# matthieugomez/LeastSquaresOptim.jl

Hardware: AMD Instinct MI355X
Metric: lm_lsmr_outer_iterations_per_sec (higher is better)
Workload: dtype f64

## Files before the change

leastsquaresoptim.jl_amd/csrc/lsq_optimize.hip:

```cpp
#include <chrono>
#include <cmath>
#include <cstring>

#include "lsq_solver.h"
#include "lsq_spmv.h"

static constexpr double MIN_DELTA = 1e-16, MAX_DELTA = 1e16, MIN_STEP_QUALITY = 1e-3;
static constexpr double MIN_DIAGONAL = 1e-6, MAX_DIAGONAL = 1e32;
static constexpr double DECREASE_THRESHOLD = 0.25, INCREASE_THRESHOLD = 0.75;

enum { SL_GRAD = 8, SL_DX = 9, SL_NONFIN = 10, SL_TRIAL = 11, SL_PRED = 12, SL_SSR = 13, SL_W0 = 14, SL_W1 = 15,
       SL_W2 = 16, SL_SUM = 17 };

extern "C" int lsq_solver_create(lsq_ctx *c, lsq_mat *J, int kind, int for_lm, lsq_solver **out) {
    LSQ_RANGE("lsq_solver_create");
    if (!c || !J || !out) return LSQ_EARG;
    if (kind == LSQ_QR && J->kind != LSQ_MAT_DENSE) {
        lsq_set_error("solver QR() is not available for sparse Jacobians. Choose between Cholesky() and LSMR()");
        return LSQ_EARG;
    }
    const bool blockdiag = kind == LSQ_CHOLESKY && J->kind == LSQ_MAT_CSC && J->bd_blocks > 0;
    const bool bordered = kind == LSQ_CHOLESKY && J->kind == LSQ_MAT_CSC && J->br_blocks > 0;
    if (kind == LSQ_CHOLESKY && J->kind != LSQ_MAT_DENSE && !blockdiag && !bordered) {
        lsq_set_error("MethodError: no AbstractAllocatedSolver for Cholesky() with a sparse Jacobian "
// ... 351 lines not shown
    });
}

__global__ void __launch_bounds__(LSQ_NT)
k_wdot_slot(int n, const double *__restrict__ x, const double *__restrict__ y, const double *__restrict__ w,
            double *partials, unsigned *counter, double *out) {
    __shared__ double sh[LSQ_NT / 64];
    double acc = 0.0;
    for (int i = blockIdx.x * LSQ_NT + threadIdx.x; i < n; i += gridDim.x * LSQ_NT) acc += w[i] * x[i] * y[i];
    double b = block_sum<LSQ_NT>(acc, sh);
    grid_reduce<LSQ_NT>(b, partials, counter, gridDim.x, sh, [=](double t) { *out = t; });
}

__global__ void __launch_bounds__(LSQ_NT)
k_lincomb(int n, double a, const double *__restrict__ p, double b, const double *__restrict__ q,
          double *__restrict__ out) {
    for (int i = blockIdx.x * LSQ_NT + threadIdx.x; i < n; i += gridDim.x * LSQ_NT) {
        double v = p[i] * a;
        if (q) v += b * q[i];
        out[i] = v;
    }
}

static inline int ngrid(const lsq_ctx *c, long long n) {
    long long g = (n + LSQ_NT - 1) / LSQ_NT;
    long long cap = (long long)c->num_cus * 8;
    if (g > cap) g = cap;
    return g < 1 ? 1 : (int)g;
}

static int sumsq_to_slot(lsq_ctx *c, bool exact, long long n, const double *x, int ctr, double *d_out,
                         LsqSlotPublish pub = LsqSlotPublish()) {
    if (exact) return lsq_seq_reduce(c, 1, (int)n, x, nullptr, nullptr, d_out);
    long long g = (n + LSQ_NT - 1) / LSQ_NT, cap = (long long)c->num_cus * 2;
    if (g > cap) g = cap;
    if (g < 1) g = 1;
    LSQ_LAUNCH(k_sumsq_slot, dim3((int)g), dim3(LSQ_NT), 0, c->stream, n, x, c->d_partials, lsq_ctr(c, ctr), d_out,
                       pub);
    return LSQ_OK;
}
static int model_f(double *out, const double *x, void *user);
static int model_g(lsq_mat *J, const double *x, void *user);
static int model_f_sumsq(void *user, double *out, const double *x, int ctr, double *d_out, LsqSlotPublish pub, bool *done,
                         const int *skip = nullptr);
struct SpecGrad {
    int *gate;
    double ssr;
    double *grad;
    bool launched;
};
static int model_pair_tail(void *user, lsq_mat *J, const double *dx, const double *fcur, double *ftrial, const double *xt,
                           double *slot_pred, double *slot_trial, LsqSlotPublish pub, const int *skip, bool *done,
                           SpecGrad *sg = nullptr);
static void model_trial_buffers(void *user, const double *xt, double **t_out, double **s_out);
static int f_then_sumsq(lsq_ctx *c, bool exact, lsq_f_callback f, void *user, long long m, double *out, const double *x, int ctr,
                        double *d_out, LsqSlotPublish pub = LsqSlotPublish(), const int *skip = nullptr) {
    if (!exact && f == model_f) {
        bool fused = false;
        if (model_f_sumsq(user, out, x, ctr, d_out, pub, &fused, skip) != 0) {
            lsq_set_error("user callback reported failure");
            return LSQ_ECALLBACK;
        }
        if (fused) return LSQ_OK;
    } else if (f(out, x, user) != 0) {
        lsq_set_error("user callback reported failure");
        return LSQ_ECALLBACK;
    }
    return sumsq_to_slot(c, exact, m, out, ctr, d_out, pub);
}
static int predicted_to_slot(lsq_ctx *c, bool exact, lsq_mat *J, const double *d, const double *f, double *scratch,
                             int ctr, double *d_out, LsqSlotPublish pub = LsqSlotPublish(), const int *skip = nullptr);
static int wdot_to_slot(lsq_ctx *c, bool exact, int n, const double *x, const double *y, const double *w, int ctr,
                        double *d_out);
static int gradient_into(lsq_ctx *c, bool exact, lsq_mat *J, const double *f, double *g);

struct LoopBuffers {
    lsq_ctx *c;
    int m, n;
    double *dx = nullptr, *dtd = nullptr, *xt = nullptr, *ftrial = nullptr;
    double *dgn = nullptr, *dgr = nullptr, *grad = nullptr, *fpred = nullptr;
    double *lo = nullptr, *hi = nullptr;
    int *gate_ring = nullptr;
    int gate_next = 0;
    static constexpr int GATE_RING = 1024;
    ~LoopBuffers() {
        hipFree(gate_ring);
        hipFree(dx); hipFree(dtd); hipFree(xt); hipFree(ftrial); hipFree(dgn); hipFree(dgr); hipFree(grad); hipFree(fpred); hipFree(lo);
        hipFree(hi);
    }
};

struct LsqWorkspace {
    lsq_mat *J = nullptr;
    int m = 0, n = 0, optimizer = -1, solver_kind = -1;
    bool has_lo = false, has_hi = false;
    LoopBuffers *buf = nullptr;
    lsq_solver *solver = nullptr;
};
void lsq_workspace_free(void *p) {
    LsqWorkspace *w = (LsqWorkspace *)p;
    if (!w) return;
    delete w->buf;
    if (w->solver) lsq_solver_destroy(w->solver);
    delete w;
}

// ... 120 lines not shown
        return LSQ_ECALLBACK;
    }
    *ssr = v[0];
    *gnorm = v[1];
    *all_converged = v[2] > 0.5 ? 1 : 0;
    return LSQ_OK;
}

struct ShardedExit {
    lsq_ctx *c;
    const lsq_options *o;
    ShardedExit(lsq_ctx *c_, const lsq_options *o_) : c(c_), o(o_) {
        t_xchg_issued = 0;
        t_xchg_hook_failed = false;
    }
    int finish(int st) {
        c->idle_hook = nullptr;
        c->idle_user = nullptr;
        if (st != LSQ_OK && st != LSQ_ERCCL && o->allreduce && !t_xchg_hook_failed && t_xchg_issued < o->iterations) {
            double v[3] = {0.0, 0.0, -1.0};
            (void)o->allreduce(v, 3, o->allreduce_user);
        }
        return st;
    }
};

#define CB(call)                                          \
    do {                                                  \
        if ((call) != 0) {                                \
            lsq_set_error("user callback reported failure"); \
            return LSQ_ECALLBACK;                         \
        }                                                 \
    } while (0)

static int call_g(lsq_g_callback g, lsq_mat *J, const double *x, void *user) {
    J->version++;
    if (J->kind == LSQ_MAT_CSC && !J->d_cs_user) J->csr_fresh = false;
    CB(g(J, x, user));
    return lsq_ensure_csr(J);
}
int lsq_call_g(lsq_g_callback g, lsq_mat *J, const double *x, void *user) { return call_g(g, J, x, user); }

struct IterateGuard {
    lsq_ctx *c;
    double *&x, *&fcur;
    double *x_user, *fcur_user;
    int m, n;
    ~IterateGuard() {
        if (x != x_user) lsq_d2d(c, x_user, x, (size_t)n * sizeof(double));
        if (fcur != fcur_user) lsq_d2d(c, fcur_user, fcur, (size_t)m * sizeof(double));
    }
};

static int start_residual(lsq_ctx *c, lsq_mat *J, lsq_f_callback f, void *user, double *fcur, const double *x, double *ssr,
                          int *nonfinite_at) {
    const int m = J->m, n = J->n;
    if (lsq_small_mat(J) || lsq_small_vec(m) || m <= 0) {
        CB(f(fcur, x, user));
        LSQ_TRY(lsq_sumsq(c, m, fcur, ssr));
        return lsq_first_nonfinite(c, n, x, nonfinite_at);
    }
    static_assert(SL_TRIAL == SL_NONFIN + 1, "the two scalars of the loop head travel together");
    LSQ_TRY(lsq_first_nonfinite_to_slot(c, n, x, c->d_slots + SL_NONFIN));
    LSQ_TRY(f_then_sumsq(c, false, f, user, m, fcur, x, 7, c->d_slots + SL_TRIAL));
    double sl[2];
    LSQ_TRY(lsq_read_slots(c, SL_NONFIN, 2, sl));
    *nonfinite_at = (int)sl[0];
    *ssr = sl[1];
    return LSQ_OK;
}

static int optimize_lm_loop(lsq_ctx *c, lsq_solver *sv, LoopBuffers &b, lsq_mat *J, double *x_user, double *fcur_user,
                            lsq_f_callback f, lsq_g_callback g, void *user, const lsq_options *o, lsq_result *r);
static int optimize_lm(lsq_ctx *c, lsq_solver *sv, LoopBuffers &b, lsq_mat *J, double *x_user, double *fcur_user,
                       lsq_f_callback f, lsq_g_callback g, void *user, const lsq_options *o, lsq_result *r) {
    ShardedExit ex{c, o};
    return ex.finish(optimize_lm_loop(c, sv, b, J, x_user, fcur_user, f, g, user, o, r));
}
static int optimize_lm_loop(lsq_ctx *c, lsq_solver *sv, LoopBuffers &b, lsq_mat *J, double *x_user, double *fcur_user,
                            lsq_f_callback f, lsq_g_callback g, void *user, const lsq_options *o, lsq_result *r) {
    const int m = J->m, n = J->n;
    double *x = x_user, *fcur = fcur_user, *xt = b.xt, *ftrial = b.ftrial;
    IterateGuard guard{c, x, fcur, x_user, fcur_user, m, n};
    double delta = o->delta > 0 ? o->delta : 10.0;
    double decrease_factor = 2.0;
    int f_calls = 0, g_calls = 0, mul_calls = 0, xc = 0, fc = 0, gc = 0;
    bool converged = false;
    double ssr;
    int iter = 0, nonfinite_at = -1;
    const bool sharded = o->row_allreduce != nullptr;
    if (sharded) CB(f(fcur, x, user));
    else LSQ_TRY(start_residual(c, J, f, user, fcur, x, &ssr, &nonfinite_at));
    f_calls++;
    auto rows_sum = [&](double *d_buf, int count) -> int {
        if (o->row_allreduce(d_buf, count, (void *)c->stream, o->row_allreduce_user) != 0) {
            lsq_set_error("row all-reduce callback reported failure");
            return LSQ_ECALLBACK;
        }
        return LSQ_OK;
    };
    if (sharded) {
        LSQ_TRY(sumsq_to_slot(c, false, m, fcur, 7, c->d_slots + SL_TRIAL));
        LSQ_TRY(rows_sum(c->d_slots + SL_TRIAL, 1));
        LSQ_TRY(lsq_read_slots(c, SL_TRIAL, 1, &ssr));
        LSQ_TRY(lsq_first_nonfinite(c, n, x, &nonfinite_at));
    }
    r->ssr0 = ssr;
    double maxabs_gr = INFINITY;
    bool need_jac = true;
    const int gn = ngrid(c, n);
    const bool exact = lsq_small_mat(J) && !sharded && !(sv->kind == LSQ_LSMR && sv->gen_ldiv);
    int last_inner = 0;
    const bool no_spec_grad = getenv("LSQ_NO_SPEC_GRADIENT") != nullptr;
    bool spec_launched = false, spec_grad_ready = false, spec_pending = false;
    struct SpecGuard { lsq_mat *J; bool &ready; bool &pending; ~SpecGuard() { if (ready || pending) lsq_sparse_colsum_forget(J); } }
        spec_guard{J, spec_grad_ready, spec_pending};
    int local_done = 0;
    double gssr = ssr, ggr = maxabs_gr;
    long long inner_total = 0;
    while (iter < o->iterations) {
        if (!o->allreduce && converged) break;
        if (o->allreduce && converged) {
            int all = 1;
            gssr = ssr; ggr = maxabs_gr;
            LSQ_TRY(global_exchange(o, &gssr, &ggr, &all));
            if (all) break;
            ++iter; local_done = 1;
            continue;
        }
        iter++;
        if (nonfinite_at >= 0) {
            r->bad_index = nonfinite_at;
            r->iterations = iter - 1;
            lsq_set_error("IsFiniteException: non-finite x at index %d", nonfinite_at);
            return LSQ_ENONFINITE;
        }
        if (need_jac) {
            LSQ_TRY(call_g(g, J, x, user));
            g_calls++;
            need_jac = false;
        }
        bool have_grad = false;
        if (spec_grad_ready) {
            lsq_sparse_grad_colsum_adopt(J);
            have_grad = true;
// ... 129 lines not shown
        const double rho = pred_red > 0 ? (ssr - trial_ssr) / pred_red : 0.0;
        const bool accepted = rho > MIN_STEP_QUALITY;
        const bool dev_accepted = spec_launched && sl[5] != 0.0;
        spec_grad_ready = spec_launched && accepted && dev_accepted;
        if (spec_launched && dev_accepted && !accepted) lsq_sparse_colsum_forget(J);
        spec_pending = false;
        converged = assess(maxabs_dx, maxabs_gr, ssr, trial_ssr, o->x_tol, o->f_tol, o->g_tol, accepted, &xc, &fc, &gc);
        if (accepted) {
            std::swap(fcur, ftrial);
            std::swap(x, xt);
            ssr = trial_ssr;
            double q = 1.0 - (2.0 * rho - 1.0) * (2.0 * rho - 1.0) * (2.0 * rho - 1.0);
            delta = std::min(delta / std::max(1.0 / 3.0, q), MAX_DELTA);
            decrease_factor = 2.0;
            need_jac = true;
            nonfinite_at = trial_nonfinite;
        } else {
            LSQ_LAUNCH(k_revert, dim3(gn), dim3(LSQ_NT), 0, c->stream, n, xt, b.dx, x);
            nonfinite_at = trial_nonfinite;
            delta = std::max(delta / decrease_factor, MIN_DELTA);
            decrease_factor *= 2.0;
        }
        record(o, c, iter, n, ssr, maxabs_gr, delta, rho, lmiter, accepted ? 1 : 0, x);
    }
    (void)local_done;
    LSQ_HIP(hipStreamSynchronize(c->stream));
    r->optimizer = LSQ_LEVENBERG_MARQUARDT;
    r->ssr = o->allreduce ? gssr : ssr;
    r->iterations = iter;
    r->converged = converged; r->x_converged = xc; r->f_converged = fc; r->g_converged = gc;
    r->f_calls = f_calls; r->g_calls = g_calls; r->mul_calls = mul_calls;
    r->lsmr_iterations = inner_total;
    return LSQ_OK;
}

static int optimize_dogleg_loop(lsq_ctx *c, lsq_solver *sv, LoopBuffers &b, lsq_mat *J, double *x, double *fcur,
                                lsq_f_callback f, lsq_g_callback g, void *user, const lsq_options *o, lsq_result *r);
static int optimize_dogleg(lsq_ctx *c, lsq_solver *sv, LoopBuffers &b, lsq_mat *J, double *x, double *fcur,
                           lsq_f_callback f, lsq_g_callback g, void *user, const lsq_options *o, lsq_result *r) {
    ShardedExit ex{c, o};
    return ex.finish(optimize_dogleg_loop(c, sv, b, J, x, fcur, f, g, user, o, r));
}
static int optimize_dogleg_loop(lsq_ctx *c, lsq_solver *sv, LoopBuffers &b, lsq_mat *J, double *x_user, double *fcur_user,
                                lsq_f_callback f, lsq_g_callback g, void *user, const lsq_options *o, lsq_result *r) {
    const int m = J->m, n = J->n;
    double *x = x_user, *fcur = fcur_user, *xt = b.xt, *ftrial = b.ftrial;
    IterateGuard guard{c, x, fcur, x_user, fcur_user, m, n};
    double delta = o->delta > 0 ? o->delta : 1.0;
    bool reuse = false, converged = false;
    double wnorm_dgn = 0.0, wnorm_dgr = 0.0, alpha = 0.0, wdot_gr_gn = 0.0;
    int f_calls = 0, g_calls = 0, mul_calls = 0, xc = 0, fc = 0, gc = 0;
    double ssr;
    int iter = 0, nonfinite_at = -1;
    LSQ_TRY(start_residual(c, J, f, user, fcur, x, &ssr, &nonfinite_at));
    f_calls++;
    r->ssr0 = ssr;
    double maxabs_gr = INFINITY;
    const int gn = ngrid(c, n);
    const bool exact = lsq_small_mat(J);
    double gssr = ssr, ggr = maxabs_gr;
    long long inner_total = 0;
    while (iter < o->iterations) {
        if (!o->allreduce && converged) break;
        if (o->allreduce && converged) {
            int all = 1;
            gssr = ssr; ggr = maxabs_gr;
            LSQ_TRY(global_exchange(o, &gssr, &ggr, &all));
            if (all) break;
            ++iter;
            continue;
        }
        iter++;
        if (nonfinite_at >= 0) {
            r->bad_index = nonfinite_at;
            r->iterations = iter - 1;
            lsq_set_error("IsFiniteException: non-finite x at index %d", nonfinite_at);
            return LSQ_ENONFINITE;
        }
        int ls_iter = 0;
        bool exchanged = false;
        if (!reuse) {
            LSQ_TRY(call_g(g, J, x, user));
            g_calls++;
            bool have_grad = false;
            if (!exact && J->colsum_version != J->version && lsq_can_fuse_grad_colsum(J)) {
                LSQ_TRY(lsq_sparse_grad_colsum(J, fcur, b.dgr));
                have_grad = true;
            }
            const double *cs = lsq_cached_colsum(J);
            if (!cs) return LSQ_EHIP;
            LSQ_LAUNCH(k_dl_scale, dim3(gn), dim3(LSQ_NT), 0, c->stream, n, cs, b.dtd);
            if (iter == 1) {
                double wx2;
                LSQ_TRY(lsq_wdot(c, n, x, x, b.dtd, &wx2));
                double wx = std::sqrt(wx2);
                if (wx > 0) delta *= wx;
            }
            if (!have_grad) LSQ_TRY(gradient_into(c, exact, J, fcur, b.dgr));
            mul_calls++;
            LSQ_LAUNCH(k_gradnorm, dim3(gn), dim3(LSQ_NT), 0, c->stream, n, b.dgr, x, b.lo, b.hi,
                               c->d_partials, lsq_ctr(c, 4), c->d_slots + SL_GRAD);
            LSQ_TRY(lsq_ediv(c, n, b.dgr, b.dtd, b.dgr));
            LSQ_TRY(wdot_to_slot(c, exact, n, b.dgr, b.dgr, b.dtd, 5, c->d_slots + SL_W0));
            LSQ_TRY(predicted_to_slot(c, exact, J, b.dgr, nullptr, b.fpred, 6, c->d_slots + SL_SUM));
            mul_calls++;
            LSQ_TRY(lsq_fill(c, n, 0.0, b.dgn));
            if (o->allreduce) {
// ... 85 lines not shown
    r->iterations = iter;
    r->converged = converged; r->x_converged = xc; r->f_converged = fc; r->g_converged = gc;
    r->f_calls = f_calls; r->g_calls = g_calls; r->mul_calls = mul_calls;
    r->lsmr_iterations = inner_total;
    return LSQ_OK;
}

extern "C" int lsq_optimize(lsq_ctx *c, int optimizer, int solver_kind, lsq_mat *J, double *x, double *fcur,
                            lsq_f_callback f, lsq_g_callback g, void *user, const lsq_options *opt, lsq_result *res) {
    LSQ_RANGE("lsq_optimize");
    if (!c || !J || !x || !fcur || !f || !g || !opt || !res) {
        lsq_set_error("lsq_optimize: null argument");
        return LSQ_EARG;
    }
    memset(res, 0, sizeof(*res));
    res->bad_index = -1;
    LSQ_HIP(hipSetDevice(c->device));
    const int n = J->n;
    if (opt->h_lower || opt->h_upper) {
        std::vector<double> hx(n);
        LSQ_TRY(lsq_d2h(c, hx.data(), x, (size_t)n * sizeof(double)));
        int st = check_start(hx.data(), n, opt);
        if (st != LSQ_OK) {
            lsq_set_error("ArgumentError: Initial guess must be within bounds.");
            res->status = st;
            return st;
        }
    }
    LsqWorkspace *w = (LsqWorkspace *)c->workspace;
    const bool lm = optimizer == LSQ_LEVENBERG_MARQUARDT;
    if (!(w && w->J == J && w->m == J->m && w->n == J->n && w->optimizer == optimizer && w->solver_kind == solver_kind &&
          w->has_lo == (opt->h_lower != nullptr) && w->has_hi == (opt->h_upper != nullptr))) {
        lsq_workspace_free(w);
        c->workspace = nullptr;
        w = new LsqWorkspace();
        int st0 = lsq_solver_create(c, J, solver_kind, lm, &w->solver);
        if (st0 != LSQ_OK) {
            delete w;
            res->status = st0;
            return st0;
        }
        w->buf = new LoopBuffers();
        st0 = alloc_loop(*w->buf, c, J->m, J->n, opt, !lm);
        if (st0 != LSQ_OK) {
            lsq_workspace_free(w);
            res->status = st0;
            return st0;
        }
        w->J = J; w->m = J->m; w->n = J->n; w->optimizer = optimizer; w->solver_kind = solver_kind;
        w->has_lo = opt->h_lower != nullptr; w->has_hi = opt->h_upper != nullptr;
        c->workspace = w;
    } else {
        const size_t nb = (size_t)(J->n > 0 ? J->n : 1) * sizeof(double);
        LSQ_HIP(hipMemsetAsync(w->buf->dx, 0, nb, c->stream));
        if (opt->h_lower) LSQ_HIP(hipMemcpyAsync(w->buf->lo, opt->h_lower, nb, hipMemcpyHostToDevice, c->stream));
        if (opt->h_upper) LSQ_HIP(hipMemcpyAsync(w->buf->hi, opt->h_upper, nb, hipMemcpyHostToDevice, c->stream));
        if (opt->h_lower || opt->h_upper) LSQ_HIP(hipStreamSynchronize(c->stream));
    }
    if (w->solver->kind == LSQ_LSMR) {
        w->solver->precond_cb = opt->preconditioner;
        w->solver->precond_user = opt->preconditioner_user;
        w->solver->gen_update = opt->precond_update;
        w->solver->gen_ldiv = opt->precond_ldiv;
        w->solver->gen_user = opt->precond_general_user;
    }
    if (opt->row_allreduce) {
        if (!lm || w->solver->kind != LSQ_LSMR || opt->allreduce || J->kind == LSQ_MAT_OP) {
            lsq_set_error("row-sharded runs (lsq_options.row_allreduce): LevenbergMarquardt(LSMR()) on stored Jacobians only, and "
                          "not together with the independent-problems exchange (lsq_options.allreduce)");
            res->status = LSQ_EARG;
            return LSQ_EARG;
        }
        LSQ_TRY(lsq_solver_set_row_allreduce(w->solver, opt->row_allreduce, opt->row_allreduce_user,
                                             opt->global_rows > 0 ? opt->global_rows : (long long)J->m));
    } else if (w->solver->kind == LSQ_LSMR) {
        LSQ_TRY(lsq_solver_set_row_allreduce(w->solver, nullptr, nullptr, 0));
    }
    auto t0 = std::chrono::steady_clock::now();
    int st = lm ? optimize_lm(c, w->solver, *w->buf, J, x, fcur, f, g, user, opt, res)
                : optimize_dogleg(c, w->solver, *w->buf, J, x, fcur, f, g, user, opt, res);
    hipStreamSynchronize(c->stream);
    res->seconds = std::chrono::duration<double>(std::chrono::steady_clock::now() - t0).count();
    res->status = st;
    return st;
}

struct lsq_model {
    lsq_ctx *ctx;
    lsq_mat *J;
    bool fused = false;
    double *d_Acsc = nullptr;
    double *d_Acsr = nullptr;
    double *d_Ab = nullptr;
    double *d_b = nullptr;
    double *d_t = nullptr;
    double *d_s = nullptr;
    double *d_sspec = nullptr;
    const double *tanh_x = nullptr;
    const double *sfac_x = nullptr;
    double *d_b_perm = nullptr;
    double *d_perm[2] = {nullptr, nullptr};
    const double *perm_of[2] = {nullptr, nullptr};
};
static void model_perm_invalidate(lsq_model *md, const double *vec) {
    for (int k = 0; k < 2; ++k)
        if (!vec || md->perm_of[k] == vec) md->perm_of[k] = nullptr;
}

__global__ void __launch_bounds__(LSQ_NT) k_tanh(int n, const double *__restrict__ x, double *__restrict__ t) {
    for (int i = blockIdx.x * LSQ_NT + threadIdx.x; i < n; i += gridDim.x * LSQ_NT) t[i] = tanh(x[i]);
}

struct EpiResidual {
    static constexpr bool REDUCE = false;
    const int *done;
    int extra_blocks;
    const double *b;
    double *out;
    double *partials;
    unsigned *counter;
    __device__ void seg(int i, double dot, double &) const { out[i] = dot - b[i]; }
    using has_pre = void;
    __device__ double pre(int i) const { return b[i]; }
    __device__ void seg_pre(int i, double dot, double bi, double &) const { out[i] = dot - bi; }
    __device__ void extra(int, double &) const {}
    __device__ void finalize(double) const {}
};

struct EpiResidualSq {
    static constexpr bool REDUCE = true;
    const int *done;
    int extra_blocks;
    const double *b;
    double *out;
    double *partials;
    unsigned *counter;
    double *slot;
    LsqSlotPublish pub;
    __device__ void seg(int i, double dot, double &racc) const { seg_pre(i, dot, b[i], racc); }
    using has_pre = void;
    __device__ double pre(int i) const { return b[i]; }
    __device__ void seg_pre(int i, double dot, double bi, double &racc) const {
        const double v = dot - bi;
        out[i] = v;
        racc += v * v;
    }
    __device__ void extra(int, double &) const {}
    __device__ void finalize(double t) const {
        *slot = t;
        if (pub.count > 0) {
            for (int i = 0; i < pub.count; ++i)
                __hip_atomic_store(pub.dst + i, pub.src + i == slot ? t : pub.src[i], __ATOMIC_RELAXED, __HIP_MEMORY_SCOPE_SYSTEM);
            __hip_atomic_store(pub.seq_word, pub.seq, __ATOMIC_RELEASE, __HIP_MEMORY_SCOPE_SYSTEM);
        }
    }
};

__global__ void __launch_bounds__(LSQ_NT)
k_scale_cols(int n, const int *__restrict__ colptr, int m_dense, const double *__restrict__ A,
             const double *__restrict__ x, double *__restrict__ out) {
    for (int j = blockIdx.x; j < n; j += gridDim.x) {
        double t = tanh(x[j]);
        double s = 1.0 - t * t;
        long long k0 = colptr ? colptr[j] : (long long)j * m_dense;
        long long k1 = colptr ? colptr[j + 1] : (long long)(j + 1) * m_dense;
        for (long long k = k0 + threadIdx.x; k < k1; k += LSQ_NT) out[k] = A[k] * s;
    }
}
__global__ void __launch_bounds__(LSQ_NT)
k_scale_dense(int m, const double *__restrict__ A, const double *__restrict__ x, double *__restrict__ out) {
    const int j = blockIdx.x;
    const double t = tanh(x[j]);
    const double sfac = 1.0 - t * t;
    const size_t base = (size_t)j * m;
    for (int i = blockIdx.y * LSQ_NT + threadIdx.x; i < m; i += gridDim.y * LSQ_NT) out[base + i] = A[base + i] * sfac;
}
__global__ void __launch_bounds__(LSQ_NT)
k_scale_csr(long long nnz, const int *__restrict__ colidx, const double *__restrict__ A, const double *__restrict__ sfac,
            double *__restrict__ out) {
    for (long long k = blockIdx.x * (long long)LSQ_NT + threadIdx.x; k < nnz; k += (long long)gridDim.x * LSQ_NT)
        out[k] = A[k] * sfac[colidx[k]];
}
__global__ void __launch_bounds__(LSQ_NT) k_tanh_sfac(int n, const double *__restrict__ x, double *__restrict__ t,
                                                      double *__restrict__ s) {
    for (int i = blockIdx.x * LSQ_NT + threadIdx.x; i < n; i += gridDim.x * LSQ_NT) {
        const double v = tanh(x[i]);
        t[i] = v;
        s[i] = 1.0 - v * v;
    }
}
__global__ void __launch_bounds__(LSQ_NT) k_sfac(int n, const double *__restrict__ x, double *__restrict__ s) {
    for (int i = blockIdx.x * LSQ_NT + threadIdx.x; i < n; i += gridDim.x * LSQ_NT) {
        double t = tanh(x[i]);
        s[i] = 1.0 - t * t;
    }
}

__global__ void __launch_bounds__(LSQ_NT)
k_scale_bcsc(int nseg, int n, const int *__restrict__ ptr, const double *__restrict__ A, const double *__restrict__ sfac,
             double *__restrict__ out) {
    const int lane = threadIdx.x & 63, per = LSQ_NT / 64;
    for (int s = blockIdx.x * per + (threadIdx.x >> 6); s < nseg; s += gridDim.x * per) {
        const double f = sfac[s % n];
        const int k1 = ptr[s + 1];
        for (int k = ptr[s] + lane; k < k1; k += 64) out[k] = A[k] * f;
    }
}

typedef double lsq_d2 __attribute__((ext_vector_type(2)));
// ... 40 lines not shown
    lsq_mat *J = md->J;
    const bool have_tanh = md->tanh_x == x;
    md->tanh_x = nullptr;
    model_perm_invalidate(md, out);
    if (!have_tanh) {
        md->sfac_x = nullptr;
        LSQ_LAUNCH(k_tanh, dim3(ngrid(c, J->n)), dim3(LSQ_NT), 0, c->stream, J->n, x, md->d_t);
    }
    EpiResidual e{nullptr, 0, md->d_b, out, nullptr, nullptr};
    if (J->kind == LSQ_MAT_CSC && J->srows.active) {
        if (launch_sell_rows(J, nullptr, md->d_t, e, md->fused ? nullptr : md->d_Acsr) != LSQ_OK) return 1;
    } else if (J->kind == LSQ_MAT_CSC) {
        LsqSegs A = J->csr;
        A.d_val = md->d_Acsr;
        if (launch_segs<false>(c, A, md->d_t, e) != LSQ_OK) return 1;
    } else {
        lsq_mat tmp = *J;
        tmp.d_dense = md->d_Acsc;
        if (launch_product(&tmp, 0, md->d_t, e) != LSQ_OK) return 1;
    }
    return hipGetLastError() == hipSuccess ? 0 : 1;
}

static void model_trial_buffers(void *user, const double *xt, double **t_out, double **s_out) {
    lsq_model *md = (lsq_model *)user;
    md->tanh_x = md->sfac_x = nullptr;
    if ((md->J->kind == LSQ_MAT_CSC && md->J->srows.active) || md->J->kind == LSQ_MAT_DENSE) {
        *t_out = md->d_t;
        *s_out = md->d_sspec;
        md->tanh_x = md->sfac_x = xt;
    }
}

static int model_f_sumsq(void *user, double *out, const double *x, int ctr, double *d_out, LsqSlotPublish pub, bool *done,
                         const int *skip) {
    lsq_model *md = (lsq_model *)user;
    lsq_ctx *c = md->ctx;
    lsq_mat *J = md->J;
    *done = false;
    if (!(J->kind == LSQ_MAT_CSC && J->srows.active)) return model_f(out, x, user);
    model_perm_invalidate(md, out);
    EpiResidualSq e{skip, 0, md->d_b, out, c->d_partials, lsq_ctr(c, ctr), d_out, pub};
    const bool have_tanh = md->tanh_x == x;
    md->tanh_x = nullptr;
    if (!have_tanh) {
        md->sfac_x = nullptr;
        LSQ_LAUNCH(k_tanh, dim3(ngrid(c, J->n)), dim3(LSQ_NT), 0, c->stream, J->n, x, md->d_t);
    }
    if (launch_sell_rows(J, nullptr, md->d_t, e, md->fused ? nullptr : md->d_Acsr) != LSQ_OK) return 1;
    *done = true;
    return hipGetLastError() == hipSuccess ? 0 : 1;
}

static int model_pair_tail(void *user, lsq_mat *J, const double *dx, const double *fcur, double *ftrial, const double *xt,
                           double *slot_pred, double *slot_trial, LsqSlotPublish pub, const int *skip, bool *done, SpecGrad *sg) {
    lsq_model *md = (lsq_model *)user;
    lsq_ctx *c = md->ctx;
    *done = false;
    if (!(md->fused && J == md->J && J->kind == LSQ_MAT_CSC && J->srows.active && J->srows.ncw == 1 && J->d_colscale &&
          J->n <= LSQ_PAIR_X_MAX && md->tanh_x == xt) || getenv("LSQ_NO_PAIR_TAIL"))
        return 0;
    const LsqSell &S = J->srows;
    const int nxpad = (J->n + 1) & ~1;
    const size_t lds = (size_t)std::max(2 * nxpad, LSQ_SELL_ROWS_MAX) * sizeof(double);
    if (lsq_set_lds(c, (const void *)k_sell_rows_pair<0>, (size_t)2 * LSQ_PAIR_X_MAX * sizeof(double)) != LSQ_OK) return 0;
    const size_t plen = (size_t)S.nslices * 64;
    const int pgrid = std::max(1, std::min(lsq_div_up((long long)plen, LSQ_NT), c->num_cus * 8));
    if (!md->d_b_perm) {
        double *pb = nullptr, *p0 = nullptr, *p1 = nullptr;
        if (hipMalloc(&pb, plen * sizeof(double)) != hipSuccess || hipMalloc(&p0, plen * sizeof(double)) != hipSuccess ||
            hipMalloc(&p1, plen * sizeof(double)) != hipSuccess) {
            (void)hipGetLastError();
            hipFree(pb); hipFree(p0); hipFree(p1);
            return 0;
        }
        md->d_b_perm = pb; md->d_perm[0] = p0; md->d_perm[1] = p1;
        LSQ_LAUNCH(k_sell_perm_rows<0>, dim3(pgrid), dim3(LSQ_NT), 0, c->stream, sell_dev(S), S.wrows, S.nslices, (const double *)md->d_b,
                   md->d_b_perm);
    }
    int k = md->perm_of[0] == fcur ? 0 : (md->perm_of[1] == fcur ? 1 : -1);
    if (k < 0) {
        k = 0;
        LSQ_LAUNCH(k_sell_perm_rows<0>, dim3(pgrid), dim3(LSQ_NT), 0, c->stream, sell_dev(S), S.wrows, S.nslices, fcur, md->d_perm[k]);
        md->perm_of[k] = fcur;
    }
    md->perm_of[1 - k] = ftrial;
    md->tanh_x = nullptr;
    const int grid = std::max(1, std::min(S.nblocks, c->num_cus));
    const bool spec = sg && sg->gate && md->sfac_x == xt;
    SellPairEpi e{skip, md->d_perm[k], md->d_b_perm, ftrial, md->d_perm[1 - k], c->d_partials, c->d_partials + 4096, lsq_ctr(c, 7),
                  slot_pred, slot_trial, pub, spec ? sg->gate : nullptr, spec ? sg->ssr : 0.0, MIN_STEP_QUALITY,
                  c->d_slots + SL_SSR};
    LSQ_LAUNCH(k_sell_rows_pair<0>, dim3(grid), dim3(LSQ_BIG_NT), lds, c->stream, sell_dev(S), S.wrows, J->m, dx, J->d_colscale,
               (const double *)md->d_t, J->n, nxpad, e);
    *done = true;
    if (hipGetLastError() != hipSuccess) return 1;
    if (spec) {
        const int st = lsq_sparse_grad_colsum_spec(J, ftrial, sg->grad, md->d_sspec, sg->gate);
        if (st == LSQ_OK) sg->launched = true;
        else if (st != LSQ_EARG) return 1;
    }
    return 0;
}

static int model_g(lsq_mat *J, const double *x, void *user) {
    lsq_model *md = (lsq_model *)user;
    lsq_ctx *c = md->ctx;
    if (J->kind == LSQ_MAT_DENSE) {}
    else if (md->sfac_x == x) std::swap(md->d_s, md->d_sspec);
    else LSQ_LAUNCH(k_sfac, dim3(ngrid(c, J->n)), dim3(LSQ_NT), 0, c->stream, J->n, x, md->d_s);
    md->sfac_x = nullptr;
    md->tanh_x = nullptr;
    if (md->fused) {
        if (lsq_mat_set_colscale(J, md->d_s) != LSQ_OK) return 1;
        return hipGetLastError() == hipSuccess ? 0 : 1;
    }
    if (J->kind == LSQ_MAT_CSC) {
        const bool have_cols = J->scols.active || J->nwin > 1;
        const unsigned short *rcol = J->srows.active ? J->srows.d_idx16 : J->csr.d_idx16;
        const unsigned short *ccol = J->scols.active ? J->scols.d_col16 : J->bcsc.d_col16;
        double *rval = J->srows.active ? J->srows.d_val : J->csr.d_val;
        double *cval = J->scols.active ? J->scols.d_val : J->bcsc.d_val;
        const long long rlen = lsq_mirror_rows_len(J), clen = lsq_mirror_cols_len(J);
        const bool lds_ok = J->n <= 12000 && J->nnz >= (1 << 20) && J->srows.ncw == 1;
        const bool lazy_csc = lds_ok && rcol && have_cols && ccol && lsq_can_fuse_grad_colsum(J);
        if (!lazy_csc) {
            int grid = J->n < c->num_cus * 16 ? (J->n > 0 ? J->n : 1) : c->num_cus * 16;
            LSQ_LAUNCH(k_scale_cols, dim3(grid), dim3(LSQ_NT), 0, c->stream, J->n, J->csc.d_ptr, 0, md->d_Acsc,
                               x, J->csc.d_val);
        }
        J->csc_fresh = !lazy_csc;
        const size_t lds = (size_t)J->n * sizeof(double);
// ... 103 lines not shown
```

leastsquaresoptim.jl_amd/csrc/lsq_sell.h:

```cpp
#pragma once

constexpr int LSQ_SELL_POS_BITS = 13;
constexpr unsigned LSQ_SELL_POS_MASK = (1u << LSQ_SELL_POS_BITS) - 1u;
constexpr int LSQ_SELL_ROWS_MAX = 4096;
constexpr int LSQ_SELL_CW_AUTO = 6;
constexpr int LSQ_SELL_CW_MAX = 32;
constexpr int LSQ_SELL_GROWS_MAX = 16384;
constexpr int LSQ_SELL_CCOLS_MAX = 2560;

struct SellDev {
    const int2 *smeta;
    const unsigned *info;
    const unsigned short *idx16;
    const double *val;
    int nblocks;
    int spw;
};

template <int U>
struct SellBatch {
    double2 a[U];
    unsigned c[U];
};
template <int U, bool CLAMP>
// ... 69 lines not shown
    if (rem > 4) {
        SellBatch<8> B;
        sell_batch_load<8, true>(B, vp, ip, p0, np);
        sell_batch_sum<8, true, SQ>(B, p0, np, len, xl, sum, sq);
    } else if (rem > 2) {
        SellBatch<4> B;
        sell_batch_load<4, true>(B, vp, ip, p0, np);
        sell_batch_sum<4, true, SQ>(B, p0, np, len, xl, sum, sq);
    } else if (rem > 0) {
        SellBatch<2> B;
        sell_batch_load<2, true>(B, vp, ip, p0, np);
        sell_batch_sum<2, true, SQ>(B, p0, np, len, xl, sum, sq);
    }
    if (TAIL && (L & 1)) sell_tail_sum<SQ>(tail, L, len, xl, sum, sq);
}

template <bool SQ>
__device__ __forceinline__ void sell_lane_sum(const double *__restrict__ vp, const unsigned short *__restrict__ ip, int L, int len,
                                              const double *xl, double &sum, double &sq, int lane) {
    sell_lane_sum_from<SQ>(vp, ip, 0, L, len, xl, sum, sq, lane);
}

struct SellSliceRef {
    int2 sm;
    unsigned inf;
};
__device__ __forceinline__ SellSliceRef sell_slice_ref(const SellDev &S, int s, int s1, int lane) {
    SellSliceRef r;
    r.sm = make_int2(0, 0);
    r.inf = LSQ_SELL_POS_MASK;
    if (s < s1) {
        r.sm = S.smeta[__builtin_amdgcn_readfirstlane(s)];
        r.inf = S.info[(size_t)s * 64 + lane];
    }
    return r;
}
template <bool SQ, class Out>
__device__ __forceinline__ void sell_wave_slices(const SellDev &S, int s0, int s1, int wv, int lane, const double *xl, Out out) {
    constexpr int NW = LSQ_BIG_NT / 64;
    int s = s0 + wv;
    SellSliceRef A = sell_slice_ref(S, s, s1, lane);
    __syncthreads();
    for (; s < s1; s += NW) {
        const SellSliceRef a = A;
        A = sell_slice_ref(S, s + NW, s1, lane);
        const size_t oa = (size_t)a.sm.x + lane * 2;
        const unsigned pos = a.inf & LSQ_SELL_POS_MASK;
        double sum = 0.0, sq = 0.0;
        sell_lane_sum<SQ>(S.val + oa, S.idx16 + oa, a.sm.y, (int)(a.inf >> LSQ_SELL_POS_BITS), xl, sum, sq, lane);
        if (pos != LSQ_SELL_POS_MASK) out(pos, sum, sq);
    }
}

template <class Epi>
__global__ void __launch_bounds__(LSQ_BIG_NT) k_sell_rows(SellDev S, int wrows, int m, const double *__restrict__ x,
                                                          const double *__restrict__ xscale, int nx, int nxpad, Epi epi) {
    extern __shared__ __attribute__((aligned(16))) double smem[];
    __shared__ double sh[LSQ_BIG_NT / 64];
    double *xl = smem;
    double *yw = smem + nxpad;
    const int tid = threadIdx.x, lane = tid & 63, wv = tid >> 6;
    constexpr int XR = (LSQ_LDS_X_MAX + LSQ_BIG_NT - 1) / LSQ_BIG_NT;
    double xr[XR];
#pragma unroll
    for (int q = 0; q < XR; ++q) xr[q] = x[min(tid + q * LSQ_BIG_NT, nx - 1)];
    if (xscale) {
        double sr[XR];
#pragma unroll
        for (int q = 0; q < XR; ++q) sr[q] = xscale[min(tid + q * LSQ_BIG_NT, nx - 1)];
#pragma unroll
        for (int q = 0; q < XR; ++q) xr[q] *= sr[q];
    }
    const int dflag = epi.done ? *epi.done : 0;

    if constexpr (EpiHasBlockPrepare<Epi>::value) epi.block_prepare();
    if constexpr (EpiHasPrepare<Epi>::value) epi.prepare();
#pragma unroll
    for (int q = 0; q < XR; ++q)
        if (tid + q * LSQ_BIG_NT < nx) xl[tid + q * LSQ_BIG_NT] = xr[q];
    if (dflag) return;
    constexpr int Q = LSQ_SELL_ROWS_MAX / LSQ_BIG_NT;
    double racc = 0.0;
    for (int w = blockIdx.x; w < S.nblocks; w += gridDim.x) {
        const int base = w * wrows, rows = min(wrows, m - base);
        const int s0 = w * S.spw, s1 = s0 + S.spw;
        double pre[Q];
        if constexpr (EpiHasPre<Epi>::value) {
#pragma unroll
            for (int q = 0; q < Q; ++q) pre[q] = epi.pre(base + min(tid + q * LSQ_BIG_NT, rows - 1));
        }
        sell_wave_slices<false>(S, s0, s1, wv, lane, xl, [&](unsigned pos, double sum, double) { yw[pos] = sum; });
        __syncthreads();
#pragma unroll
        for (int q = 0; q < Q; ++q) {
            const int i = tid + q * LSQ_BIG_NT;
            if (i < rows) {
                if constexpr (EpiHasPre<Epi>::value) epi.seg_pre(base + i, yw[i], pre[q], racc);
                else epi.seg(base + i, yw[i], racc);
            }
        }
    }
    for (int e = blockIdx.x; e < epi.extra_blocks; e += gridDim.x)
        if (tid < LSQ_NT) epi.extra(e, racc);
    finish_block_nt<LSQ_BIG_NT>(epi, racc, sh);
}

template <int U, bool CLAMP>
__device__ __forceinline__ void sell_batch_sum2(SellBatch<U> &B, int p0, int np, int len, const double *xa, const double *xb,
                                                double &sa, double &sb) {
#pragma unroll
    for (int u = 0; u < U; ++u) {
        const unsigned i0 = B.c[u] & 0xffffu, i1 = B.c[u] >> 16;
        double a0 = B.a[u].x * xa[i0], a1 = B.a[u].y * xa[i1], b0 = B.a[u].x * xb[i0], b1 = B.a[u].y * xb[i1];
        asm volatile("" : "+v"(a0), "+v"(a1), "+v"(b0), "+v"(b1));
        const int j = 2 * (p0 + u);
        const bool pin = !CLAMP || p0 + u < np;
        const bool in0 = pin && j < len, in1 = pin && j + 1 < len;
        const double ta0 = sa + a0;
        sa = in0 ? ta0 : sa;
        const double ta1 = sa + a1;
        sa = in1 ? ta1 : sa;
        const double tb0 = sb + b0;
        sb = in0 ? tb0 : sb;
        const double tb1 = sb + b1;
        sb = in1 ? tb1 : sb;
    }
}
__device__ __forceinline__ void sell_lane_sum2(const double *__restrict__ vp, const unsigned short *__restrict__ ip, int L, int len,
                                               const double *xa, const double *xb, double &sa, double &sb, int lane) {
    const int np = L >> 1;
    int p0 = 0;
    SellTail tail;
    tail.a = 0.0;
    tail.c = 0;
    if (L & 1) tail = sell_tail_load(vp, ip, L, lane);
    for (; p0 + 8 <= np; p0 += 8) {
        SellBatch<8> B;
        sell_batch_load<8, false>(B, vp, ip, p0, np);
        sell_batch_sum2<8, false>(B, p0, np, len, xa, xb, sa, sb);
    }
    const int rem = np - p0;
    if (rem > 4) {
        SellBatch<8> B;
        sell_batch_load<8, true>(B, vp, ip, p0, np);
        sell_batch_sum2<8, true>(B, p0, np, len, xa, xb, sa, sb);
    } else if (rem > 2) {
        SellBatch<4> B;
        sell_batch_load<4, true>(B, vp, ip, p0, np);
        sell_batch_sum2<4, true>(B, p0, np, len, xa, xb, sa, sb);
    } else if (rem > 0) {
        SellBatch<2> B;
// ... 299 lines not shown
```

Before: 4053.

## Fuse model start residual with tanh, nonfinite check, dx zeroing and permuted output

Adds a dedicated start kernel for the built-in model that computes tanh and its derivative for x, zeros dx, and reduces the nonfinite index in one launch, replacing a separate memset and nonfinite pass. The initial residual SpMV can also write a slice-permuted copy of the residual, so the first paired-tail iteration does not need a separate permutation pass. This adds another epilogue variant to the SELL kernel and more state-tracking coupling between start and tail paths. The work only happens once per solve, so the gain is per-solve launch overhead.

```diff
diff --git a/leastsquaresoptim.jl_amd/csrc/lsq_optimize.hip b/leastsquaresoptim.jl_amd/csrc/lsq_optimize.hip
--- a/leastsquaresoptim.jl_amd/csrc/lsq_optimize.hip
+++ b/leastsquaresoptim.jl_amd/csrc/lsq_optimize.hip
@@ -427,6 +427,10 @@
 static int model_pair_tail(void *user, lsq_mat *J, const double *dx, const double *fcur, double *ftrial, const double *xt,
                            double *slot_pred, double *slot_trial, LsqSlotPublish pub, const int *skip, bool *done,
                            SpecGrad *sg = nullptr);
+static bool model_start_applies(lsq_f_callback f, void *user, const lsq_mat *J);
+static int model_start(void *user, double *fcur, const double *x, double *dx0, bool pair_tail, double *slot_nonfin,
+                       double *slot_ssr, LsqSlotPublish pub);
+static void model_solve_over(void *user);
 static void model_trial_buffers(void *user, const double *xt, double **t_out, double **s_out);
 static int f_then_sumsq(lsq_ctx *c, bool exact, lsq_f_callback f, void *user, long long m, double *out, const double *x, int ctr,
                         double *d_out, LsqSlotPublish pub = LsqSlotPublish(), const int *skip = nullptr) {
@@ -653,8 +657,8 @@
     }
 };
 
-static int start_residual(lsq_ctx *c, lsq_mat *J, lsq_f_callback f, void *user, double *fcur, const double *x, double *ssr,
-                          int *nonfinite_at) {
+static int start_residual(lsq_ctx *c, lsq_mat *J, lsq_f_callback f, void *user, double *fcur, const double *x, double *dx0,
+                          bool pair_tail, double *ssr, int *nonfinite_at) {
     const int m = J->m, n = J->n;
     if (lsq_small_mat(J) || lsq_small_vec(m) || m <= 0) {
         CB(f(fcur, x, user));
@@ -662,9 +666,17 @@
         return lsq_first_nonfinite(c, n, x, nonfinite_at);
     }
     static_assert(SL_TRIAL == SL_NONFIN + 1, "the two scalars of the loop head travel together");
+    double sl[2];
+    if (model_start_applies(f, user, J)) {
+        const LsqSlotPublish pub = lsq_slots_ticket(c, SL_NONFIN, 2);
+        CB(model_start(user, fcur, x, dx0, pair_tail, c->d_slots + SL_NONFIN, c->d_slots + SL_TRIAL, pub));
+        LSQ_TRY(lsq_wait_slots(c, SL_NONFIN, 2, pub.seq, sl));
+        *nonfinite_at = (int)sl[0];
+        *ssr = sl[1];
+        return LSQ_OK;
+    }
     LSQ_TRY(lsq_first_nonfinite_to_slot(c, n, x, c->d_slots + SL_NONFIN));
     LSQ_TRY(f_then_sumsq(c, false, f, user, m, fcur, x, 7, c->d_slots + SL_TRIAL));
-    double sl[2];
     LSQ_TRY(lsq_read_slots(c, SL_NONFIN, 2, sl));
     *nonfinite_at = (int)sl[0];
     *ssr = sl[1];
@@ -691,7 +703,7 @@
     int iter = 0, nonfinite_at = -1;
     const bool sharded = o->row_allreduce != nullptr;
     if (sharded) CB(f(fcur, x, user));
-    else LSQ_TRY(start_residual(c, J, f, user, fcur, x, &ssr, &nonfinite_at));
+    else LSQ_TRY(start_residual(c, J, f, user, fcur, x, b.dx, sv->kind == LSQ_LSMR && !b.lo && !b.hi, &ssr, &nonfinite_at));
     f_calls++;
     auto rows_sum = [&](double *d_buf, int count) -> int {
         if (o->row_allreduce(d_buf, count, (void *)c->stream, o->row_allreduce_user) != 0) {
@@ -927,7 +939,7 @@
     int f_calls = 0, g_calls = 0, mul_calls = 0, xc = 0, fc = 0, gc = 0;
     double ssr;
     int iter = 0, nonfinite_at = -1;
-    LSQ_TRY(start_residual(c, J, f, user, fcur, x, &ssr, &nonfinite_at));
+    LSQ_TRY(start_residual(c, J, f, user, fcur, x, b.dx, false, &ssr, &nonfinite_at));
     f_calls++;
     r->ssr0 = ssr;
     double maxabs_gr = INFINITY;
@@ -1119,7 +1131,7 @@
         c->workspace = w;
     } else {
         const size_t nb = (size_t)(J->n > 0 ? J->n : 1) * sizeof(double);
-        LSQ_HIP(hipMemsetAsync(w->buf->dx, 0, nb, c->stream));
+        if (opt->row_allreduce || !model_start_applies(f, user, J)) LSQ_HIP(hipMemsetAsync(w->buf->dx, 0, nb, c->stream));
         if (opt->h_lower) LSQ_HIP(hipMemcpyAsync(w->buf->lo, opt->h_lower, nb, hipMemcpyHostToDevice, c->stream));
         if (opt->h_upper) LSQ_HIP(hipMemcpyAsync(w->buf->hi, opt->h_upper, nb, hipMemcpyHostToDevice, c->stream));
         if (opt->h_lower || opt->h_upper) LSQ_HIP(hipStreamSynchronize(c->stream));
@@ -1146,6 +1158,7 @@
     auto t0 = std::chrono::steady_clock::now();
     int st = lm ? optimize_lm(c, w->solver, *w->buf, J, x, fcur, f, g, user, opt, res)
                 : optimize_dogleg(c, w->solver, *w->buf, J, x, fcur, f, g, user, opt, res);
+    if (f == model_f) model_solve_over(user);
     hipStreamSynchronize(c->stream);
     res->seconds = std::chrono::duration<double>(std::chrono::steady_clock::now() - t0).count();
     res->status = st;
@@ -1222,6 +1235,37 @@
         }
     }
 };
+
+struct EpiResidualSqPerm : EpiResidualSq {
+    double *out_perm;
+    using has_slice_out = void;
+    __device__ double seg_pre_keep(int i, double dot, double bi, double &racc) const {
+        const double v = dot - bi;
+        out[i] = v;
+        racc += v * v;
+        return v;
+    }
+    __device__ void slice_out(size_t k, double v) const { out_perm[k] = v; }
+};
+
+__global__ void __launch_bounds__(LSQ_NT)
+k_model_start(int n, const double *__restrict__ x, double *__restrict__ t_out, double *__restrict__ s_out, double *__restrict__ dx0,
+              double *partials, unsigned *counter, double *out_nonfin) {
+    __shared__ double sh[LSQ_NT / 64];
+    double code = 0.0;
+    for (int i = blockIdx.x * LSQ_NT + threadIdx.x; i < n; i += gridDim.x * LSQ_NT) {
+        const double v = x[i];
+        const double th = tanh(v);
+        t_out[i] = th;
+        s_out[i] = 1.0 - th * th;
+        if (dx0) dx0[i] = 0.0;
+        if (!isfinite(v) && code == 0.0) code = 1e15 - (double)(i + 1);
+    }
+    const double bv = block_max<LSQ_NT>(code, sh);
+    grid_reduce<LSQ_NT, true>(bv, partials, counter, gridDim.x, sh, [=](double t) {
+        *out_nonfin = (t == 0.0) ? -1.0 : (1e15 - t) - 1.0;
+    });
+}
 
 __global__ void __launch_bounds__(LSQ_NT)
 k_scale_cols(int n, const int *__restrict__ colptr, int m_dense, const double *__restrict__ A,
@@ -1368,32 +1412,74 @@
     return hipGetLastError() == hipSuccess ? 0 : 1;
 }
 
+static bool model_pairable(const lsq_model *md, const lsq_mat *J) {
+    return md->fused && J == md->J && J->kind == LSQ_MAT_CSC && J->srows.active && J->srows.ncw == 1 && J->d_colscale &&
+           J->n <= LSQ_PAIR_X_MAX && !getenv("LSQ_NO_PAIR_TAIL");
+}
+static bool model_perm_buffers(lsq_model *md) {
+    if (md->d_b_perm) return true;
+    lsq_ctx *c = md->ctx;
+    const LsqSell &S = md->J->srows;
+    const size_t plen = (size_t)S.nslices * 64;
+    const int pgrid = std::max(1, std::min(lsq_div_up((long long)plen, LSQ_NT), c->num_cus * 8));
+    double *pb = nullptr, *p0 = nullptr, *p1 = nullptr;
+    if (hipMalloc(&pb, plen * sizeof(double)) != hipSuccess || hipMalloc(&p0, plen * sizeof(double)) != hipSuccess ||
+        hipMalloc(&p1, plen * sizeof(double)) != hipSuccess) {
+        (void)hipGetLastError();
+        hipFree(pb); hipFree(p0); hipFree(p1);
+        return false;
+    }
+    md->d_b_perm = pb; md->d_perm[0] = p0; md->d_perm[1] = p1;
+    LSQ_LAUNCH(k_sell_perm_rows<0>, dim3(pgrid), dim3(LSQ_NT), 0, c->stream, sell_dev(S), S.wrows, S.nslices, (const double *)md->d_b,
+               md->d_b_perm);
+    return true;
+}
+
+static bool model_start_applies(lsq_f_callback f, void *user, const lsq_mat *J) {
+    if (f != model_f || !user) return false;
+    const lsq_model *md = (const lsq_model *)user;
+    return md->J == J && J->kind == LSQ_MAT_CSC && J->srows.active && J->n > 0 && J->m > 0 && !lsq_small_mat(J) &&
+           !lsq_small_vec(J->m);
+}
+static int model_start(void *user, double *fcur, const double *x, double *dx0, bool pair_tail, double *slot_nonfin,
+                       double *slot_ssr, LsqSlotPublish pub) {
+    lsq_model *md = (lsq_model *)user;
+    lsq_ctx *c = md->ctx;
+    lsq_mat *J = md->J;
+    LSQ_LAUNCH(k_model_start, dim3(ngrid(c, J->n)), dim3(LSQ_NT), 0, c->stream, J->n, x, md->d_t, md->d_sspec, dx0, c->d_partials,
+               lsq_ctr(c, 0), slot_nonfin);
+    md->tanh_x = nullptr;
+    md->sfac_x = x;
+    model_perm_invalidate(md, fcur);
+    const double *val = md->fused ? nullptr : md->d_Acsr;
+    const EpiResidualSq e{nullptr, 0, md->d_b, fcur, c->d_partials, lsq_ctr(c, 7), slot_ssr, pub};
+    if (pair_tail && model_pairable(md, J) && model_perm_buffers(md)) {
+        EpiResidualSqPerm ep{e, md->d_perm[0]};
+        if (launch_sell_rows(J, nullptr, md->d_t, ep, val) != LSQ_OK) return 1;
+        md->perm_of[0] = fcur;
+        if (md->perm_of[1] == fcur) md->perm_of[1] = nullptr;
+    } else if (launch_sell_rows(J, nullptr, md->d_t, e, val) != LSQ_OK) return 1;
+    return hipGetLastError() == hipSuccess ? 0 : 1;
+}
+
+static void model_solve_over(void *user) {
+    lsq_model *md = (lsq_model *)user;
+    md->tanh_x = md->sfac_x = nullptr;
+}
+
 static int model_pair_tail(void *user, lsq_mat *J, const double *dx, const double *fcur, double *ftrial, const double *xt,
                            double *slot_pred, double *slot_trial, LsqSlotPublish pub, const int *skip, bool *done, SpecGrad *sg) {
     lsq_model *md = (lsq_model *)user;
     lsq_ctx *c = md->ctx;
     *done = false;
-    if (!(md->fused && J == md->J && J->kind == LSQ_MAT_CSC && J->srows.active && J->srows.ncw == 1 && J->d_colscale &&
-          J->n <= LSQ_PAIR_X_MAX && md->tanh_x == xt) || getenv("LSQ_NO_PAIR_TAIL"))
-        return 0;
+    if (!(model_pairable(md, J) && md->tanh_x == xt)) return 0;
     const LsqSell &S = J->srows;
     const int nxpad = (J->n + 1) & ~1;
     const size_t lds = (size_t)std::max(2 * nxpad, LSQ_SELL_ROWS_MAX) * sizeof(double);
     if (lsq_set_lds(c, (const void *)k_sell_rows_pair<0>, (size_t)2 * LSQ_PAIR_X_MAX * sizeof(double)) != LSQ_OK) return 0;
     const size_t plen = (size_t)S.nslices * 64;
     const int pgrid = std::max(1, std::min(lsq_div_up((long long)plen, LSQ_NT), c->num_cus * 8));
-    if (!md->d_b_perm) {
-        double *pb = nullptr, *p0 = nullptr, *p1 = nullptr;
-        if (hipMalloc(&pb, plen * sizeof(double)) != hipSuccess || hipMalloc(&p0, plen * sizeof(double)) != hipSuccess ||
-            hipMalloc(&p1, plen * sizeof(double)) != hipSuccess) {
-            (void)hipGetLastError();
-            hipFree(pb); hipFree(p0); hipFree(p1);
-            return 0;
-        }
-        md->d_b_perm = pb; md->d_perm[0] = p0; md->d_perm[1] = p1;
-        LSQ_LAUNCH(k_sell_perm_rows<0>, dim3(pgrid), dim3(LSQ_NT), 0, c->stream, sell_dev(S), S.wrows, S.nslices, (const double *)md->d_b,
-                   md->d_b_perm);
-    }
+    if (!model_perm_buffers(md)) return 0;
     int k = md->perm_of[0] == fcur ? 0 : (md->perm_of[1] == fcur ? 1 : -1);
     if (k < 0) {
         k = 0;
diff --git a/leastsquaresoptim.jl_amd/csrc/lsq_sell.h b/leastsquaresoptim.jl_amd/csrc/lsq_sell.h
--- a/leastsquaresoptim.jl_amd/csrc/lsq_sell.h
+++ b/leastsquaresoptim.jl_amd/csrc/lsq_sell.h
@@ -145,6 +145,10 @@
     }
 }
 
+template <class E, class = void>
+struct EpiHasSliceOut : std::false_type {};
+template <class E>
+struct EpiHasSliceOut<E, std::void_t<typename E::has_slice_out>> : std::true_type {};
 template <class Epi>
 __global__ void __launch_bounds__(LSQ_BIG_NT) k_sell_rows(SellDev S, int wrows, int m, const double *__restrict__ x,
                                                           const double *__restrict__ xscale, int nx, int nxpad, Epi epi) {
@@ -188,8 +192,16 @@
         for (int q = 0; q < Q; ++q) {
             const int i = tid + q * LSQ_BIG_NT;
             if (i < rows) {
-                if constexpr (EpiHasPre<Epi>::value) epi.seg_pre(base + i, yw[i], pre[q], racc);
+                if constexpr (EpiHasSliceOut<Epi>::value) yw[i] = epi.seg_pre_keep(base + i, yw[i], pre[q], racc);
+                else if constexpr (EpiHasPre<Epi>::value) epi.seg_pre(base + i, yw[i], pre[q], racc);
                 else epi.seg(base + i, yw[i], racc);
+            }
+        }
+        if constexpr (EpiHasSliceOut<Epi>::value) {
+            __syncthreads();
+            for (int k = s0 * 64 + tid; k < s1 * 64; k += LSQ_BIG_NT) {
+                const unsigned pos = S.info[k] & LSQ_SELL_POS_MASK;
+                epi.slice_out((size_t)k, pos != LSQ_SELL_POS_MASK ? yw[pos] : 0.0);
             }
         }
     }
```

Result: no change. 4033 (-0.5%).
